# pmorenoz/HetMOGP

Hardware: AMD Instinct MI355X
Metric: ELBO-steps/sec (one step = ELBO + all parameter gradients) (higher is better)
Workload: dtype f64

## Files before the change

### __graft_entry__.py

```python
import os
import subprocess
import sys

ROOT = os.path.dirname(os.path.abspath(__file__))
CSRC = os.path.join(ROOT, "hetmogp_amd", "csrc")


def build():
    jobs = str(min(8, os.cpu_count() or 1))
    subprocess.run(["make", "-C", CSRC, "-j", jobs], check=True)
    probes = os.path.join(ROOT, "tools", "probes")
    os.makedirs(os.path.join(probes, "build"), exist_ok=True)
    for name in ("probe_mfma", "probe_coissue", "probe_gemm8", "probe_gemm16", "probe_gemm_abl", "probe_gemm_bdirect", "probe_i8"):
        r = subprocess.run(["/opt/rocm/bin/hipcc", "--offload-arch=gfx950", "-O3", "-Wno-unused-value",
                            os.path.join(probes, name + ".hip"), "-o", os.path.join(probes, "build", name)], check=False)
        if r.returncode != 0:
            print("build(): diagnostic probe %s did not compile (not part of libhetmogp_hip.so)" % name, file=sys.stderr)
    if ROOT not in sys.path:
        sys.path.insert(0, ROOT)
    import hetmogp_amd
    from hetmogp_amd import _lib
    assert os.path.exists(_lib.LIB_PATH)


def smoke():
    if ROOT not in sys.path:
        sys.path.insert(0, ROOT)
    import numpy as np
    from hetmogp_amd.engine import Engine
    from hetmogp_amd.synthetic import make_case
    from oracle import svmogp_oracle as so

    specs = [("Gaussian", {"sigma": 0.5}), ("Bernoulli", {}), ("Poisson", {}), ("Gamma", {})]
    for M, N in ((64, 2000), (128, 20000)):
        prm, X, Y = make_case(specs, [N] * 4, M=M, Q=3, P=1, seed=7)
        prob = so.make_problem(specs, 3, M, 1)
        want = so.elbo_grad_fused(prm, prob, X, Y)
        e = Engine(specs, 3, M, 1, device=0)
        e.set_data(X, Y)
        out = e.elbo_grad(**prm)
        worst = 0.0
        for k in ("elbo", "g_m_u", "g_L_u", "g_variance", "g_lengthscale", "g_W", "g_kappa", "g_Z"):
            a, b = np.asarray(out[k], float), np.asarray(want[k], float)
            err = float(np.max(np.abs(a - b)) / (np.max(np.abs(b)) + 1e-300))
            worst = max(worst, err)
            assert err < 1e-8, (M, k, err)
        ms, _ = e.timings()
        print("smoke OK (M=%d, N_t=%d): ELBO %.6f (oracle %.6f), worst relative error %.2e, %.2f ms on device" %
              (M, N, out["elbo"], want["elbo"], worst, ms["total"]))
        e.close()
    g = np.load(os.path.join(ROOT, "tests", "golden", "lad_h_mix_M128_ladder.npz"))
    prm, prob, X, Y, bs = so.load_case(g)
    e = Engine(prob["specs"], prob["Q"], prob["M"], prob["P"], device=0, strict_qf=True)
    e.set_data(X, Y)
    out = e.elbo_grad(batch_scale=bs, **prm)
    assert out["rungs"] == [int(r) for r in g["rungs"]], out["rungs"]
    worst = 0.0
    for k in ("elbo", "g_m_u", "g_L_u", "g_variance", "g_lengthscale", "g_W", "g_kappa", "g_Z"):
        a, b = np.asarray(out[k], float).ravel(), np.asarray(g[k], float).ravel()
        ex = float(np.max(np.abs(a - b) / (1e-5 * np.abs(b) + 1e-9 * np.max(np.abs(b)))))
        worst = max(worst, ex)
        assert ex <= 1.0, ("strict mode vs reference run", k, ex)
    print("smoke OK (strict q(f), M=128, jitter rung %s as in the reference run): worst element-wise excess over 1e-5 criterion %.3f" %
          (out["rungs"], worst))
    from hetmogp_amd import _lib
    oe = e.elbo_grad(batch_scale=bs, group_mask=_lib.GROUP_QU, **prm)
    worst_e = 0.0
    for k in ("elbo", "g_m_u", "g_L_u"):
        a, b = np.asarray(oe[k], float).ravel(), np.asarray(g[k], float).ravel()
        ex = float(np.max(np.abs(a - b) / (1e-5 * np.abs(b) + 1e-9 * np.max(np.abs(b)))))
        worst_e = max(worst_e, ex)
        assert ex <= 1.0, ("strict E-step (one-solve form) vs reference run", k, ex)
    print("smoke OK (strict E-step, one-solve form): worst element-wise excess %.3f" % worst_e)
    e.close()


if __name__ == "__main__":
    build()
    if len(sys.argv) > 1 and sys.argv[1] == "smoke":
        smoke()
```

### hetmogp_amd/csrc/gemm_rowpass.hip

```cpp
#include <cstdlib>

#include "common.h"

namespace {

constexpr int BM = 128, BN = 128, BK = 16, W = 8, NT = W * 64;
constexpr int KM_LD = 144, RM_LD = 18, TILE_DOUBLES = BK * KM_LD;
constexpr int NB = 2, WN = 32, NWN = 4;
constexpr int BK32 = 32, A32_LD = 34, BD_D = 2;

struct Tile {
  double a[2][TILE_DOUBLES];
  double b[2][TILE_DOUBLES];
};

__device__ __forceinline__ int diag_wm(int w) { return (0x4B >> w) & 1; }
__device__ __forceinline__ int diag_wn(int w) { return (0x7E84 >> (2 * w)) & 3; }

template <int ROLE, bool FOLD = false, bool BD = false>
__device__ __forceinline__ void rowpass_tile(const GemmArgs& g, int tiles_n, int ti, int tj, int split, Tile& lds, double* epi_a,
                                             int* hwinfo = nullptr) {
  const int batch = blockIdx.z;
  const int M = g.M, N = g.N, K = g.K;
  const int i0 = ti * BM, j0 = tj * BN;
  if (i0 >= M || j0 >= N) return;
  int wlo = 0;
  if (ROLE == 1 && g.b_tri > 0) wlo = j0;
  const int ksteps = (K - wlo + BK - 1) / BK;
  const int per = (ksteps + g.ksplit - 1) / g.ksplit;
  const int kbeg = wlo + split * per * BK;
  const int kend = min(K, kbeg + per * BK);

  const double* __restrict__ A = g.A + (long long)batch * g.sA;
  const double* __restrict__ B = g.B + (long long)batch * g.sB;
  const double* __restrict__ S = (ROLE == 2) ? g.kscale + (long long)batch * g.sS : nullptr;
  double* __restrict__ C = g.C + (long long)batch * g.sC + (long long)split * g.sSplit;
  double* fs_part = (ROLE == 1 && g.fs_part) ? g.fs_part + (long long)batch * g.fs_sPart : nullptr;

  const int t = threadIdx.x, lane = t & 63, w = __builtin_amdgcn_readfirstlane(t >> 6);
  const int lr = lane & 15, lk = lane >> 4;
  int wm = w >> 2, wn = w & 3;
  if (FOLD && w >= 4) wn = 3 - wn;
  const int klive = FOLD ? j0 + 32 * wn : 0;
  unsigned sub = 0xFFu;
  const bool diag = ROLE == 2 && ti == tj && g.lower_only;
  if (diag && hwinfo) {
    if (lane == 0) {
      const unsigned hw = __builtin_amdgcn_s_getreg(4 | (0 << 6) | (31 << 11));
      hwinfo[w] = (int)((hw >> 4) & 3u);
      if (w == 0) hwinfo[8] = (int)((hw >> 1) & 1u);
    }
  }
  constexpr bool SWAP = (ROLE == 1);
  const int blr = SWAP ? 4 * (lr & 3) + (lr >> 2) : lr;

  f64x4 acc[4][NB];
#pragma unroll
  for (int a = 0; a < 4; ++a)
#pragma unroll
    for (int b = 0; b < NB; ++b) acc[a][b] = f64x4{0.0, 0.0, 0.0, 0.0};

  const int ar = t >> 2, ak = (t & 3) * 4, bk = t >> 5, bc = (t & 31) * 2;
  const double* pa;
  const double* pb;
  if (ROLE == 1) {
    pa = A + (long long)min(i0 + ar, M - 1) * g.lda + ak;
    pb = B + (long long)bk * g.ldb + j0 + bc;
  } else {
    pa = A + i0 + bc;
    pb = B + j0 + bc;
  }
  double ra[4], rb[4], ks = 1.0;
  auto load = [&](int k0) {
    if (ROLE == 1) {
      const f64x2 x0 = *reinterpret_cast<const f64x2*>(pa + k0), x1 = *reinterpret_cast<const f64x2*>(pa + k0 + 2);
      ra[0] = x0.x, ra[1] = x0.y, ra[2] = x1.x, ra[3] = x1.y;
      const double* q = pb + (long long)k0 * g.ldb;
      const f64x2 y0 = *reinterpret_cast<const f64x2*>(q), y1 = *reinterpret_cast<const f64x2*>(q + 64);
      rb[0] = y0.x, rb[1] = y0.y, rb[2] = y1.x, rb[3] = y1.y;
    } else {
      const int row = k0 + bk;
      const long long off = (long long)min(row, K - 1) * g.lda;
      const f64x2 x0 = *reinterpret_cast<const f64x2*>(pa + off), x1 = *reinterpret_cast<const f64x2*>(pa + off + 64);
      ra[0] = x0.x, ra[1] = x0.y, ra[2] = x1.x, ra[3] = x1.y;
      const f64x2 y0 = *reinterpret_cast<const f64x2*>(pb + off), y1 = *reinterpret_cast<const f64x2*>(pb + off + 64);
      rb[0] = y0.x, rb[1] = y0.y, rb[2] = y1.x, rb[3] = y1.y;
      ks = (row < kend) ? S[row] : 0.0;
    }
  };
  auto stage = [&](int buf) {
    if (ROLE == 1) {
      double* sa = &lds.a[buf][ar * RM_LD + ak];
      *reinterpret_cast<f64x2*>(sa) = f64x2{ra[0], ra[1]};
      *reinterpret_cast<f64x2*>(sa + 2) = f64x2{ra[2], ra[3]};
    } else {
      double* sa = &lds.a[buf][bk * KM_LD + bc];
      *reinterpret_cast<f64x2*>(sa) = f64x2{ra[0], ra[1]};
      *reinterpret_cast<f64x2*>(sa + 64) = f64x2{ra[2], ra[3]};
#pragma unroll
      for (int i = 0; i < 4; ++i) rb[i] *= ks;
    }
    double* sb = &lds.b[buf][bk * KM_LD + bc];
    *reinterpret_cast<f64x2*>(sb) = f64x2{rb[0], rb[1]};
    *reinterpret_cast<f64x2*>(sb + 64) = f64x2{rb[2], rb[3]};
  };
  double fa[2][4], fb[2][NB];
  auto frag = [&](int buf, int kk, int s) {
    const double* fpa = (ROLE == 1) ? &lds.a[buf][(wm * 64 + lr) * RM_LD + kk * 4 + lk] : &lds.a[buf][(kk * 4 + lk) * KM_LD + wm * 64 + lr];
    const double* fpb = &lds.b[buf][(kk * 4 + lk) * KM_LD + wn * WN + blr];
#pragma unroll
    for (int i = 0; i < 4; ++i) fa[s][i] = fpa[i * 16 * (ROLE == 1 ? RM_LD : 1)];
#pragma unroll
    for (int i = 0; i < NB; ++i) fb[s][i] = fpb[i * 16];
  };
  auto mm8 = [&](int s) {
#pragma unroll
    for (int a = 0; a < 4; ++a)
#pragma unroll
      for (int b = 0; b < NB; ++b) {
        if (ROLE == 2 && !((sub >> (a * NB + b)) & 1u)) continue;
        acc[a][b] = SWAP ? __builtin_amdgcn_mfma_f64_16x16x4f64(fb[s][b], fa[s][a], acc[a][b], 0, 0, 0)
                         : __builtin_amdgcn_mfma_f64_16x16x4f64(fa[s][a], fb[s][b], acc[a][b], 0, 0, 0);
      }
  };

  if constexpr (BD) {
    static_assert(ROLE == 1 && !FOLD, "B direct: the plain forward only");
    constexpr int KS = BK32 / 4, NA = BK32 / 4;
    static_assert(KS % BD_D == 0, "static ring slots");
    static_assert(2 * BM * A32_LD <= 4 * TILE_DOUBLES, "A image at BK = 32 fits the tile buffers");
    double* const img = &lds.a[0][0];
    const int ar32 = t >> 2, ak32 = (t & 3) * 4;
    const double* pa32 = A + (long long)min(i0 + ar32, M - 1) * g.lda + ak32;
    double r32[NA];
    auto load32 = [&](int k0) {
      k0 = min(k0, kend - BK32);
#pragma unroll
      for (int i = 0; i < NA / 2; ++i) {
        const f64x2 x = *reinterpret_cast<const f64x2*>(pa32 + k0 + (i >> 1) * 16 + (i & 1) * 2);
        r32[2 * i] = x.x, r32[2 * i + 1] = x.y;
      }
    };
    auto stage32 = [&](int buf) {
      double* sa = img + buf * (BM * A32_LD) + ar32 * A32_LD + ak32;
#pragma unroll
      for (int i = 0; i < NA / 2; ++i) *reinterpret_cast<f64x2*>(sa + (i >> 1) * 16 + (i & 1) * 2) = f64x2{r32[2 * i], r32[2 * i + 1]};
    };
    const __amdgpu_buffer_rsrc_t brs = __builtin_amdgcn_make_buffer_rsrc(
        const_cast<double*>(B), 0, (int)(sizeof(double) * ((long long)(K - 1) * g.ldb + N)), 0x00020000);
    const int bvo = (int)sizeof(double) * (lk * g.ldb + j0 + wn * WN + blr);
    double gb[BD_D][NB];
    auto bload = [&](int k, int slot) {
      const int so = __builtin_amdgcn_readfirstlane(min(k, kend - 4) * g.ldb * (int)sizeof(double));
#pragma unroll
      for (int b = 0; b < NB; ++b)
        gb[slot][b] = __builtin_bit_cast(double, __builtin_amdgcn_raw_buffer_load_b64(brs, bvo + b * 16 * (int)sizeof(double), so, 0));
    };
    double ga[2][4];
    auto frag32 = [&](int buf, int kk, int s) {
      const double* fpa = img + buf * (BM * A32_LD) + (wm * 64 + lr) * A32_LD + kk * 4 + lk;
#pragma unroll
      for (int i = 0; i < 4; ++i) ga[s][i] = fpa[i * 16 * A32_LD];
    };
    auto mm32 = [&](int s, int slot) {
#pragma unroll
      for (int a = 0; a < 4; ++a)
#pragma unroll
        for (int b = 0; b < NB; ++b) acc[a][b] = __builtin_amdgcn_mfma_f64_16x16x4f64(gb[slot][b], ga[s][a], acc[a][b], 0, 0, 0);
    };
    int cur = 0;
    if (kbeg < kend) {
      load32(kbeg);
      stage32(0);
      load32(kbeg + BK32);
#pragma unroll
      for (int d = 0; d < BD_D; ++d) bload(kbeg + 4 * d, d);
    }
    __syncthreads();
    if (kbeg < kend) frag32(0, 0, 0);
    for (int k0 = kbeg; k0 < kend; k0 += BK32) {
      const bool more = k0 + BK32 < kend;
#pragma unroll
      for (int kk = 0; kk < KS; ++kk) {
        if (kk < KS - 1) {
          frag32(cur, kk + 1, (kk + 1) & 1);
        } else {
          __syncthreads();
          if (more) frag32(cur ^ 1, 0, 0);
        }
        __builtin_amdgcn_sched_barrier(0);
        mm32(kk & 1, kk % BD_D);
        __builtin_amdgcn_sched_barrier(0);
        bload(k0 + 4 * (kk + BD_D), kk % BD_D);
        if (kk == 0) {
          if (more) stage32(cur ^ 1);
          load32(k0 + 2 * BK32);
        }
        __builtin_amdgcn_sched_barrier(0);
      }
      cur ^= 1;
    }
  }

  int cur = 0;
  if (!BD && kbeg < kend) {
    load(kbeg);
    stage(0);
    if (kbeg + BK < kend) load(kbeg + BK);
  }
  if (!BD) __syncthreads();
  if (diag) {
    int role = w;
    if (hwinfo) {
      bool ok = true;
      unsigned seen = 0;
#pragma unroll
      for (int i = 0; i < 4; ++i) {
        ok = ok && hwinfo[i] == hwinfo[i + 4];
        seen |= 1u << hwinfo[i];
      }
      if (ok && seen == 0xFu) role = ((hwinfo[w] + 2 * hwinfo[8]) & 3) + (w & 4);
    }
    role = __builtin_amdgcn_readfirstlane(role);
    wm = diag_wm(role), wn = diag_wn(role);
    sub = 0;
#pragma unroll
    for (int a = 0; a < 4; ++a)
#pragma unroll
      for (int b = 0; b < NB; ++b)
        if (wn * NB + b <= wm * 4 + a) sub |= 1u << (a * NB + b);
  }
  const bool live = ROLE == 1 || sub != 0;
  if (ROLE == 2) {
    for (int k0 = kbeg; k0 < kend; k0 += BK) {
      if (k0 + BK < kend) stage(cur ^ 1);
      if (k0 + 2 * BK < kend) load(k0 + 2 * BK);
      if (live) {
#pragma unroll
        for (int kk = 0; kk < BK / 4; ++kk) {
          frag(cur, kk, 0);
          mm8(0);
        }
      }
      __syncthreads();
      cur ^= 1;
    }
  }
  if (ROLE == 1 && !BD && kbeg < kend && (!FOLD || kbeg >= klive)) frag(0, 0, 0);
#define HM_SB __builtin_amdgcn_sched_barrier(0)
  for (int k0 = kbeg; ROLE == 1 && !BD && k0 < kend; k0 += BK) {
    const bool more = k0 + BK < kend;
    const bool lv = !FOLD || k0 >= klive;
    if (lv) {
      frag(cur, 1, 1);
      HM_SB;
      mm8(0);
      HM_SB;
    }
    if (more) stage(cur ^ 1);
    if (k0 + 2 * BK < kend) load(k0 + 2 * BK);
    HM_SB;
    if (lv) {
      frag(cur, 2, 0);
      HM_SB;
      mm8(1);
      HM_SB;
      frag(cur, 3, 1);
      HM_SB;
      mm8(0);
      HM_SB;
    }
    __syncthreads();
    if (more && (!FOLD || k0 + BK >= klive)) frag(cur ^ 1, 0, 0);
    if (lv) {
      HM_SB;
      mm8(1);
      HM_SB;
    }
    cur ^= 1;
  }
#undef HM_SB

  if (ROLE == 1 && fs_part && g.fs_sq) {
#pragma unroll
    for (int a = 0; a < 4; ++a) {
      double sq = 0.0;
#pragma unroll
      for (int b = 0; b < NB; ++b)
#pragma unroll
        for (int r = 0; r < 4; ++r) sq = fma(acc[a][b][r], acc[a][b][r], sq);
      sq += __shfl_xor(sq, 16, 64);
      sq += __shfl_xor(sq, 32, 64);
      const int rl = wm * 64 + a * 16 + lr;
      if (lk == 0 && i0 + rl < M) fs_part[((long long)NWN * tiles_n + NWN * tj + wn) * M + (i0 + rl)] = sq;
    }
    if (!g.store_c) return;
  } else if (ROLE == 1 && fs_part) {
    constexpr int NCH = 2 * NB, WSTAGE = 2 * NCH * 128;
    double* flat = &lds.a[0][0];
    double* stg = flat + w * WSTAGE;
    static_assert(W * WSTAGE <= 4 * TILE_DOUBLES, "epilogue scratch fits the tile buffers");
    const int colq = j0 + wn * WN + 4 * lk;
    const double* __restrict__ Ke = g.fs_k ? g.fs_k + (long long)batch * g.sA : A;
    auto issue = [&](int a) {
      const int grow = min(i0 + wm * 64 + a * 16 + lr, M - 1);
      const double* src = Ke + (long long)grow * g.lda + colq;
      double* dst = stg + (a & 1) * (NCH * 128);
#pragma unroll
      for (int c = 0; c < NCH; ++c)
        __builtin_amdgcn_global_load_lds((const void __attribute__((address_space(1)))*)(src + (c >> 1) * 16 + (c & 1) * 2),
                                         (void __attribute__((address_space(3)))*)(dst + c * 128), 16, 0, 0);
    };
    issue(0);
    issue(1);
    if (t < 128) epi_a[t] = g.fs_a[(long long)batch * g.fs_sA + j0 + t];
    __syncthreads();
#pragma unroll
    for (int a = 0; a < 4; ++a) {
      if (a < 3) asm volatile("s_waitcnt vmcnt(4)" ::: "memory");
      else asm volatile("s_waitcnt vmcnt(0)" ::: "memory");
      const int rl = wm * 64 + a * 16 + lr;
      double sp = 0.0, sc = 0.0;
#pragma unroll
      for (int b = 0; b < NB; ++b) {
        const int cl = wn * WN + b * 16 + 4 * lk;
        const double* kp = stg + (a & 1) * (NCH * 128) + (2 * b) * 128 + 2 * lane;
        const f64x2 k01 = *reinterpret_cast<const f64x2*>(kp), k23 = *reinterpret_cast<const f64x2*>(kp + 128);
        const double kv[4] = {k01.x, k01.y, k23.x, k23.y};
        const f64x2 a01 = *reinterpret_cast<const f64x2*>(epi_a + cl), a23 = *reinterpret_cast<const f64x2*>(epi_a + cl + 2);
        const double av[4] = {a01.x, a01.y, a23.x, a23.y};
#pragma unroll
        for (int r = 0; r < 4; ++r) {
          sp += kv[r] * av[r];
          sc += acc[a][b][r] * kv[r];
        }
      }
#pragma unroll
      for (int o = 16; o <= 32; o <<= 1) {
        sp += __shfl_xor(sp, o, 64);
        sc += __shfl_xor(sc, o, 64);
      }
      if (lk == 0 && i0 + rl < M) {
        double* o = fs_part + ((long long)(NWN * tj + wn)) * M + (i0 + rl);
        const long long ss = (long long)NWN * tiles_n * M;
        o[0] = sp, o[ss] = sc;
      }
      if (a < 2) {
        asm volatile("" ::: "memory");
        issue(a + 2);
      }
    }
    if (!g.store_c) return;
  }
  if (SWAP) {
#pragma unroll
    for (int a = 0; a < 4; ++a) {
      const int row = i0 + wm * 64 + a * 16 + lr;
      if (row >= M) continue;
      double* crow = C + (long long)row * g.ldc + j0 + wn * WN + 4 * lk;
      if (g.c_sub) {
        const double* srow = g.c_src ? g.c_src + (long long)batch * g.sC + (long long)row * g.ldc + j0 + wn * WN + 4 * lk : crow;
#pragma unroll
        for (int b = 0; b < NB; ++b) {
          const f64x2 c01 = *reinterpret_cast<const f64x2*>(srow + b * 16), c23 = *reinterpret_cast<const f64x2*>(srow + b * 16 + 2);
          *reinterpret_cast<f64x2*>(crow + b * 16) = f64x2{c01.x - acc[a][b][0], c01.y - acc[a][b][1]};
          *reinterpret_cast<f64x2*>(crow + b * 16 + 2) = f64x2{c23.x - acc[a][b][2], c23.y - acc[a][b][3]};
        }
        continue;
      }
#pragma unroll
      for (int b = 0; b < NB; ++b) {
        *reinterpret_cast<f64x2*>(crow + b * 16) = f64x2{acc[a][b][0], acc[a][b][1]};
        *reinterpret_cast<f64x2*>(crow + b * 16 + 2) = f64x2{acc[a][b][2], acc[a][b][3]};
      }
    }
    return;
  }
#pragma unroll
  for (int a = 0; a < 4; ++a)
#pragma unroll
    for (int r = 0; r < 4; ++r) {
      double* crow = C + (long long)(i0 + wm * 64 + a * 16 + 4 * r + lk) * g.ldc + j0 + wn * WN + lr;
#pragma unroll
      for (int b = 0; b < NB; ++b)
        if ((sub >> (a * NB + b)) & 1u) crow[b * 16] = acc[a][b][r];
    }
}

template <int ROLE, bool PAIR, bool BD = false>
__device__ __forceinline__ void rowpass_block(const GemmArgs& g, int tiles_n, int ntiles, Tile& lds, double* epi_a,
                                              int* hwinfo = nullptr) {

  int v = blockIdx.x, split = 0;
  int ti, tj;
  if (ROLE == 2 && g.lower_only) {
    const int T = tiles_n, noff = T * (T - 1) / 2, ks8 = (g.ksplit > 1) ? ((g.ksplit + 7) / 8) * 8 : 1, gx1 = noff * ks8;
    if (v < gx1) {
      int u = v;
      if (g.ksplit > 1) {
        const int xcd = v & 7, idx = v >> 3;
        split = (idx / noff) * 8 + xcd;
        u = idx % noff;
      }
      ti = (int)((sqrt(8.0 * (double)u + 1.0) + 1.0) * 0.5);
      while (ti * (ti + 1) / 2 <= u) ++ti;
      while (ti * (ti - 1) / 2 > u) --ti;
      tj = u - ti * (ti - 1) / 2;
    } else {
      const int u = v - gx1;
      split = u / T;
      ti = tj = u - split * T;
    }
    if (split >= g.ksplit) return;
  } else {
    if (g.ksplit > 1) {
      const int xcd = v & 7, idx = v >> 3;
      split = (idx / ntiles) * 8 + xcd;
      v = idx % ntiles;
      if (split >= g.ksplit) return;
    } else if ((ntiles & 7) == 0) {
      const int cpx = ntiles >> 3;
      v = (v & 7) * cpx + (v >> 3);
    }
    const int tcols = PAIR ? tiles_n / 2 : tiles_n;
    ti = v / tcols;
    tj = v - ti * tcols;
  }
  rowpass_tile<ROLE, PAIR, BD>(g, tiles_n, ti, tj, split, lds, epi_a, hwinfo);
  if (PAIR) {
    __syncthreads();
    rowpass_tile<ROLE, PAIR>(g, tiles_n, ti, tiles_n - 1 - tj, split, lds, epi_a);
  }
}

template <int ROLE>
__global__ __launch_bounds__(NT, 4) void rowpass_gemm_kernel(GemmArgs g, int tiles_n, int ntiles) {
  __shared__ __attribute__((aligned(16))) Tile lds;
  __shared__ __attribute__((aligned(16))) double epi_a[ROLE == 1 ? 128 : 2];
  __shared__ int hwinfo[ROLE == 2 ? 16 : 1];
  rowpass_block<ROLE, false, ROLE == 1>(g, tiles_n, ntiles, lds, epi_a, ROLE == 2 ? hwinfo : nullptr);
}
__global__ __launch_bounds__(NT, 4) void rowpass_fwd_staged_kernel(GemmArgs g, int tiles_n, int ntiles) {
  __shared__ __attribute__((aligned(16))) Tile lds;
  __shared__ __attribute__((aligned(16))) double epi_a[128];
  rowpass_block<1, false>(g, tiles_n, ntiles, lds, epi_a);
}
__global__ __launch_bounds__(NT, 4) void rowpass_fold_pair_kernel(GemmArgs g, int tiles_n, int ntiles) {
  __shared__ __attribute__((aligned(16))) Tile lds;
  __shared__ __attribute__((aligned(16))) double epi_a[128];
  rowpass_block<1, true>(g, tiles_n, ntiles, lds, epi_a);
}

bool aligned16(const void* p) { return (((uintptr_t)p) & 15) == 0; }

}

bool gemm_rowpass_eligible(const GemmArgs& g) {
  const bool sub = g.role == 1 && g.alpha == -1.0 && g.beta == 1.0 && !g.fs_part && g.b_tri == 0 && g.store_c;
  if (g.nouter != 1 || (!sub && (g.alpha != 1.0 || g.beta != 0.0)) || g.win || g.M_last || g.N_last || g.K_last || g.a_tri) return false;
  if ((g.lda & 1) || (g.ldb & 1) || (g.ldc & 1) || !aligned16(g.A) || !aligned16(g.B) || !aligned16(g.C)) return false;
  if (g.c_src && (!sub || !aligned16(g.c_src))) return false;
  if (g.fs_k && (g.role != 1 || !g.fs_part || g.fs_sq || !aligned16(g.fs_k))) return false;
  if ((g.sA & 1) || (g.sB & 1) || (g.sC & 1) || (g.sSplit & 1)) return false;
  if (g.role == 1)
    return !g.a_kmajor && g.b_kmajor && !g.lower_only && g.ksplit == 1 && !g.kscale && g.b_tri >= 0 && (g.N % BN) == 0 &&
           (g.K % BK) == 0 && (g.K == g.N || sub) && g.K >= BK && g.M >= 1;
  if (g.role == 2)
    return g.a_kmajor && g.b_kmajor && g.kscale && g.b_tri == 0 && g.M == g.N && (g.N % BN) == 0 &&
           g.lda == g.ldb && g.K >= 1;
  return false;
}

void launch_gemm_rowpass(const GemmArgs& g_in, hipStream_t stream) {
  GemmArgs g = g_in;
  g.c_sub = (g.role == 1 && g.alpha == -1.0 && g.beta == 1.0) ? 1 : 0;
  const int tiles_m = (g.M + BM - 1) / BM, tiles_n = (g.N + BN - 1) / BN;
  const int ntiles = g.lower_only ? tiles_m * (tiles_m + 1) / 2 : tiles_m * tiles_n;
  const int gx = (g.ksplit > 1) ? ntiles * ((g.ksplit + 7) / 8) * 8 : ntiles;
  dim3 grid(gx, 1, g.nbatch);
  if (g.role == 1) {
    const int pair = (g.b_tri > 0 && g.ksplit == 1 && tiles_n >= 2 && (tiles_n & 1) == 0) ? 1 : 0;
    if (pair) {
      grid.x = tiles_m * (tiles_n / 2);
      hipLaunchKernelGGL(rowpass_fold_pair_kernel, grid, dim3(NT), 0, stream, g, tiles_n, (int)grid.x);
    } else if (!g.c_sub && g.b_tri == 0 && (g.K % BK32) == 0 && ((long long)(g.K - 1) * g.ldb + g.N) * (long long)sizeof(double) <= 0x7FFFFFFFLL) {
      hipLaunchKernelGGL((rowpass_gemm_kernel<1>), grid, dim3(NT), 0, stream, g, tiles_n, ntiles);
    } else {
      hipLaunchKernelGGL(rowpass_fwd_staged_kernel, grid, dim3(NT), 0, stream, g, tiles_n, ntiles);
    }
  } else {
    hipLaunchKernelGGL((rowpass_gemm_kernel<2>), grid, dim3(NT), 0, stream, g, tiles_n, ntiles);
  }
}

int launch_gemm_rowpass_or_general(const GemmArgs& g, hipStream_t stream) {
  const bool eligible = gemm_rowpass_eligible(g);
  if ((g.fs_sq || g.fs_k) && !eligible)
    throw HipError{hipErrorInvalidValue, "fs_sq / fs_k are features of the specialised forward kernel only", __FILE__, __LINE__};
  if (eligible) {
    launch_gemm_rowpass(g, stream);
    return NWN;
  }
  if (g.role == 1 && (g.alpha != 1.0 || g.beta != 0.0)) {
    GemmArgs h = g;
    h.role = 0;
    launch_gemm_f64(h, stream);
    return 2;
  }
  launch_gemm_f64(g, stream);
  return 2;
}
```

Measured before the change: 8.497.

## Replace role-2 Gram GEMM path with direct-A buffer-load gram tile kernel

The scaled Gram (role 2) GEMM is moved out of the shared row-pass tile into a dedicated gram_tile routine. Each wave now owns one 16-row strip and keeps up to 8 accumulators. A fragments are read straight from global memory through buffer loads in a small ring, and only the scaled B panel is staged in LDS at BK=32. Diagonal tiles give each wave a triangular share of the work instead of relying on the old hardware-ID based role mapping. This is meant to cut LDS traffic and wasted MFMAs on lower-triangular tiles, at the cost of global-load latency on A and a new 32-bit offset limit added to the eligibility check.

```diff
diff --git a/__graft_entry__.py b/__graft_entry__.py
--- a/__graft_entry__.py
+++ b/__graft_entry__.py
@@ -11,7 +11,7 @@
     subprocess.run(["make", "-C", CSRC, "-j", jobs], check=True)
     probes = os.path.join(ROOT, "tools", "probes")
     os.makedirs(os.path.join(probes, "build"), exist_ok=True)
-    for name in ("probe_mfma", "probe_coissue", "probe_gemm8", "probe_gemm16", "probe_gemm_abl", "probe_gemm_bdirect", "probe_i8"):
+    for name in ("probe_mfma", "probe_coissue", "probe_gemm8", "probe_gemm16", "probe_gemm_abl", "probe_gemm_bdirect", "probe_gram_direct", "probe_i8"):
         r = subprocess.run(["/opt/rocm/bin/hipcc", "--offload-arch=gfx950", "-O3", "-Wno-unused-value",
                             os.path.join(probes, name + ".hip"), "-o", os.path.join(probes, "build", name)], check=False)
         if r.returncode != 0:
diff --git a/hetmogp_amd/csrc/gemm_rowpass.hip b/hetmogp_amd/csrc/gemm_rowpass.hip
--- a/hetmogp_amd/csrc/gemm_rowpass.hip
+++ b/hetmogp_amd/csrc/gemm_rowpass.hip
@@ -8,24 +8,23 @@
 constexpr int KM_LD = 144, RM_LD = 18, TILE_DOUBLES = BK * KM_LD;
 constexpr int NB = 2, WN = 32, NWN = 4;
 constexpr int BK32 = 32, A32_LD = 34, BD_D = 2;
+constexpr int GB = 8, GBG = 4, G_D = 2;
 
 struct Tile {
   double a[2][TILE_DOUBLES];
   double b[2][TILE_DOUBLES];
 };
 
-__device__ __forceinline__ int diag_wm(int w) { return (0x4B >> w) & 1; }
-__device__ __forceinline__ int diag_wn(int w) { return (0x7E84 >> (2 * w)) & 3; }
-
-template <int ROLE, bool FOLD = false, bool BD = false>
-__device__ __forceinline__ void rowpass_tile(const GemmArgs& g, int tiles_n, int ti, int tj, int split, Tile& lds, double* epi_a,
-                                             int* hwinfo = nullptr) {
+__device__ __forceinline__ int diag_wm(int w) { return w < 4 ? 7 - w : w - 4; }
+
+template <bool FOLD = false, bool BD = false>
+__device__ __forceinline__ void rowpass_tile(const GemmArgs& g, int tiles_n, int ti, int tj, int split, Tile& lds, double* epi_a) {
   const int batch = blockIdx.z;
   const int M = g.M, N = g.N, K = g.K;
   const int i0 = ti * BM, j0 = tj * BN;
   if (i0 >= M || j0 >= N) return;
   int wlo = 0;
-  if (ROLE == 1 && g.b_tri > 0) wlo = j0;
+  if (g.b_tri > 0) wlo = j0;
   const int ksteps = (K - wlo + BK - 1) / BK;
   const int per = (ksteps + g.ksplit - 1) / g.ksplit;
   const int kbeg = wlo + split * per * BK;
@@ -33,26 +32,16 @@
 
   const double* __restrict__ A = g.A + (long long)batch * g.sA;
   const double* __restrict__ B = g.B + (long long)batch * g.sB;
-  const double* __restrict__ S = (ROLE == 2) ? g.kscale + (long long)batch * g.sS : nullptr;
   double* __restrict__ C = g.C + (long long)batch * g.sC + (long long)split * g.sSplit;
-  double* fs_part = (ROLE == 1 && g.fs_part) ? g.fs_part + (long long)batch * g.fs_sPart : nullptr;
+  double* fs_part = g.fs_part ? g.fs_part + (long long)batch * g.fs_sPart : nullptr;
 
   const int t = threadIdx.x, lane = t & 63, w = __builtin_amdgcn_readfirstlane(t >> 6);
   const int lr = lane & 15, lk = lane >> 4;
-  int wm = w >> 2, wn = w & 3;
+  const int wm = w >> 2;
+  int wn = w & 3;
   if (FOLD && w >= 4) wn = 3 - wn;
   const int klive = FOLD ? j0 + 32 * wn : 0;
-  unsigned sub = 0xFFu;
-  const bool diag = ROLE == 2 && ti == tj && g.lower_only;
-  if (diag && hwinfo) {
-    if (lane == 0) {
-      const unsigned hw = __builtin_amdgcn_s_getreg(4 | (0 << 6) | (31 << 11));
-      hwinfo[w] = (int)((hw >> 4) & 3u);
-      if (w == 0) hwinfo[8] = (int)((hw >> 1) & 1u);
-    }
-  }
-  constexpr bool SWAP = (ROLE == 1);
-  const int blr = SWAP ? 4 * (lr & 3) + (lr >> 2) : lr;
+  const int blr = 4 * (lr & 3) + (lr >> 2);
 
   f64x4 acc[4][NB];
 #pragma unroll
@@ -61,55 +50,30 @@
     for (int b = 0; b < NB; ++b) acc[a][b] = f64x4{0.0, 0.0, 0.0, 0.0};
 
   const int ar = t >> 2, ak = (t & 3) * 4, bk = t >> 5, bc = (t & 31) * 2;
-  const double* pa;
-  const double* pb;
-  if (ROLE == 1) {
-    pa = A + (long long)min(i0 + ar, M - 1) * g.lda + ak;
-    pb = B + (long long)bk * g.ldb + j0 + bc;
-  } else {
-    pa = A + i0 + bc;
-    pb = B + j0 + bc;
-  }
-  double ra[4], rb[4], ks = 1.0;
+  const double* pa = A + (long long)min(i0 + ar, M - 1) * g.lda + ak;
+  const double* pb = B + (long long)bk * g.ldb + j0 + bc;
+  double ra[4], rb[4];
   auto load = [&](int k0) {
-    if (ROLE == 1) {
-      const f64x2 x0 = *reinterpret_cast<const f64x2*>(pa + k0), x1 = *reinterpret_cast<const f64x2*>(pa + k0 + 2);
-      ra[0] = x0.x, ra[1] = x0.y, ra[2] = x1.x, ra[3] = x1.y;
-      const double* q = pb + (long long)k0 * g.ldb;
-      const f64x2 y0 = *reinterpret_cast<const f64x2*>(q), y1 = *reinterpret_cast<const f64x2*>(q + 64);
-      rb[0] = y0.x, rb[1] = y0.y, rb[2] = y1.x, rb[3] = y1.y;
-    } else {
-      const int row = k0 + bk;
-      const long long off = (long long)min(row, K - 1) * g.lda;
-      const f64x2 x0 = *reinterpret_cast<const f64x2*>(pa + off), x1 = *reinterpret_cast<const f64x2*>(pa + off + 64);
-      ra[0] = x0.x, ra[1] = x0.y, ra[2] = x1.x, ra[3] = x1.y;
-      const f64x2 y0 = *reinterpret_cast<const f64x2*>(pb + off), y1 = *reinterpret_cast<const f64x2*>(pb + off + 64);
-      rb[0] = y0.x, rb[1] = y0.y, rb[2] = y1.x, rb[3] = y1.y;
-      ks = (row < kend) ? S[row] : 0.0;
-    }
+    const f64x2 x0 = *reinterpret_cast<const f64x2*>(pa + k0), x1 = *reinterpret_cast<const f64x2*>(pa + k0 + 2);
+    ra[0] = x0.x, ra[1] = x0.y, ra[2] = x1.x, ra[3] = x1.y;
+    const double* q = pb + (long long)k0 * g.ldb;
+    const f64x2 y0 = *reinterpret_cast<const f64x2*>(q), y1 = *reinterpret_cast<const f64x2*>(q + 64);
+    rb[0] = y0.x, rb[1] = y0.y, rb[2] = y1.x, rb[3] = y1.y;
   };
   auto stage = [&](int buf) {
-    if (ROLE == 1) {
-      double* sa = &lds.a[buf][ar * RM_LD + ak];
-      *reinterpret_cast<f64x2*>(sa) = f64x2{ra[0], ra[1]};
-      *reinterpret_cast<f64x2*>(sa + 2) = f64x2{ra[2], ra[3]};
-    } else {
-      double* sa = &lds.a[buf][bk * KM_LD + bc];
-      *reinterpret_cast<f64x2*>(sa) = f64x2{ra[0], ra[1]};
-      *reinterpret_cast<f64x2*>(sa + 64) = f64x2{ra[2], ra[3]};
-#pragma unroll
-      for (int i = 0; i < 4; ++i) rb[i] *= ks;
-    }
+    double* sa = &lds.a[buf][ar * RM_LD + ak];
+    *reinterpret_cast<f64x2*>(sa) = f64x2{ra[0], ra[1]};
+    *reinterpret_cast<f64x2*>(sa + 2) = f64x2{ra[2], ra[3]};
     double* sb = &lds.b[buf][bk * KM_LD + bc];
     *reinterpret_cast<f64x2*>(sb) = f64x2{rb[0], rb[1]};
     *reinterpret_cast<f64x2*>(sb + 64) = f64x2{rb[2], rb[3]};
   };
   double fa[2][4], fb[2][NB];
   auto frag = [&](int buf, int kk, int s) {
-    const double* fpa = (ROLE == 1) ? &lds.a[buf][(wm * 64 + lr) * RM_LD + kk * 4 + lk] : &lds.a[buf][(kk * 4 + lk) * KM_LD + wm * 64 + lr];
+    const double* fpa = &lds.a[buf][(wm * 64 + lr) * RM_LD + kk * 4 + lk];
     const double* fpb = &lds.b[buf][(kk * 4 + lk) * KM_LD + wn * WN + blr];
 #pragma unroll
-    for (int i = 0; i < 4; ++i) fa[s][i] = fpa[i * 16 * (ROLE == 1 ? RM_LD : 1)];
+    for (int i = 0; i < 4; ++i) fa[s][i] = fpa[i * 16 * RM_LD];
 #pragma unroll
     for (int i = 0; i < NB; ++i) fb[s][i] = fpb[i * 16];
   };
@@ -117,15 +81,11 @@
 #pragma unroll
     for (int a = 0; a < 4; ++a)
 #pragma unroll
-      for (int b = 0; b < NB; ++b) {
-        if (ROLE == 2 && !((sub >> (a * NB + b)) & 1u)) continue;
-        acc[a][b] = SWAP ? __builtin_amdgcn_mfma_f64_16x16x4f64(fb[s][b], fa[s][a], acc[a][b], 0, 0, 0)
-                         : __builtin_amdgcn_mfma_f64_16x16x4f64(fa[s][a], fb[s][b], acc[a][b], 0, 0, 0);
-      }
+      for (int b = 0; b < NB; ++b) acc[a][b] = __builtin_amdgcn_mfma_f64_16x16x4f64(fb[s][b], fa[s][a], acc[a][b], 0, 0, 0);
   };
 
   if constexpr (BD) {
-    static_assert(ROLE == 1 && !FOLD, "B direct: the plain forward only");
+    static_assert(!FOLD, "B direct: the plain forward only");
     constexpr int KS = BK32 / 4, NA = BK32 / 4;
     static_assert(KS % BD_D == 0, "static ring slots");
     static_assert(2 * BM * A32_LD <= 4 * TILE_DOUBLES, "A image at BK = 32 fits the tile buffers");
@@ -209,46 +169,9 @@
     if (kbeg + BK < kend) load(kbeg + BK);
   }
   if (!BD) __syncthreads();
-  if (diag) {
-    int role = w;
-    if (hwinfo) {
-      bool ok = true;
-      unsigned seen = 0;
-#pragma unroll
-      for (int i = 0; i < 4; ++i) {
-        ok = ok && hwinfo[i] == hwinfo[i + 4];
-        seen |= 1u << hwinfo[i];
-      }
-      if (ok && seen == 0xFu) role = ((hwinfo[w] + 2 * hwinfo[8]) & 3) + (w & 4);
-    }
-    role = __builtin_amdgcn_readfirstlane(role);
-    wm = diag_wm(role), wn = diag_wn(role);
-    sub = 0;
-#pragma unroll
-    for (int a = 0; a < 4; ++a)
-#pragma unroll
-      for (int b = 0; b < NB; ++b)
-        if (wn * NB + b <= wm * 4 + a) sub |= 1u << (a * NB + b);
-  }
-  const bool live = ROLE == 1 || sub != 0;
-  if (ROLE == 2) {
-    for (int k0 = kbeg; k0 < kend; k0 += BK) {
-      if (k0 + BK < kend) stage(cur ^ 1);
-      if (k0 + 2 * BK < kend) load(k0 + 2 * BK);
-      if (live) {
-#pragma unroll
-        for (int kk = 0; kk < BK / 4; ++kk) {
-          frag(cur, kk, 0);
-          mm8(0);
-        }
-      }
-      __syncthreads();
-      cur ^= 1;
-    }
-  }
-  if (ROLE == 1 && !BD && kbeg < kend && (!FOLD || kbeg >= klive)) frag(0, 0, 0);
+  if (!BD && kbeg < kend && (!FOLD || kbeg >= klive)) frag(0, 0, 0);
 #define HM_SB __builtin_amdgcn_sched_barrier(0)
-  for (int k0 = kbeg; ROLE == 1 && !BD && k0 < kend; k0 += BK) {
+  for (int k0 = kbeg; !BD && k0 < kend; k0 += BK) {
     const bool more = k0 + BK < kend;
     const bool lv = !FOLD || k0 >= klive;
     if (lv) {
@@ -281,7 +204,7 @@
   }
 #undef HM_SB
 
-  if (ROLE == 1 && fs_part && g.fs_sq) {
+  if (fs_part && g.fs_sq) {
 #pragma unroll
     for (int a = 0; a < 4; ++a) {
       double sq = 0.0;
@@ -295,7 +218,7 @@
       if (lk == 0 && i0 + rl < M) fs_part[((long long)NWN * tiles_n + NWN * tj + wn) * M + (i0 + rl)] = sq;
     }
     if (!g.store_c) return;
-  } else if (ROLE == 1 && fs_part) {
+  } else if (fs_part) {
     constexpr int NCH = 2 * NB, WSTAGE = 2 * NCH * 128;
     double* flat = &lds.a[0][0];
     double* stg = flat + w * WSTAGE;
@@ -352,44 +275,142 @@
     }
     if (!g.store_c) return;
   }
-  if (SWAP) {
-#pragma unroll
-    for (int a = 0; a < 4; ++a) {
-      const int row = i0 + wm * 64 + a * 16 + lr;
-      if (row >= M) continue;
-      double* crow = C + (long long)row * g.ldc + j0 + wn * WN + 4 * lk;
-      if (g.c_sub) {
-        const double* srow = g.c_src ? g.c_src + (long long)batch * g.sC + (long long)row * g.ldc + j0 + wn * WN + 4 * lk : crow;
-#pragma unroll
-        for (int b = 0; b < NB; ++b) {
-          const f64x2 c01 = *reinterpret_cast<const f64x2*>(srow + b * 16), c23 = *reinterpret_cast<const f64x2*>(srow + b * 16 + 2);
-          *reinterpret_cast<f64x2*>(crow + b * 16) = f64x2{c01.x - acc[a][b][0], c01.y - acc[a][b][1]};
-          *reinterpret_cast<f64x2*>(crow + b * 16 + 2) = f64x2{c23.x - acc[a][b][2], c23.y - acc[a][b][3]};
+#pragma unroll
+  for (int a = 0; a < 4; ++a) {
+    const int row = i0 + wm * 64 + a * 16 + lr;
+    if (row >= M) continue;
+    double* crow = C + (long long)row * g.ldc + j0 + wn * WN + 4 * lk;
+    if (g.c_sub) {
+      const double* srow = g.c_src ? g.c_src + (long long)batch * g.sC + (long long)row * g.ldc + j0 + wn * WN + 4 * lk : crow;
+#pragma unroll
+      for (int b = 0; b < NB; ++b) {
+        const f64x2 c01 = *reinterpret_cast<const f64x2*>(srow + b * 16), c23 = *reinterpret_cast<const f64x2*>(srow + b * 16 + 2);
+        *reinterpret_cast<f64x2*>(crow + b * 16) = f64x2{c01.x - acc[a][b][0], c01.y - acc[a][b][1]};
+        *reinterpret_cast<f64x2*>(crow + b * 16 + 2) = f64x2{c23.x - acc[a][b][2], c23.y - acc[a][b][3]};
+      }
+      continue;
+    }
+#pragma unroll
+    for (int b = 0; b < NB; ++b) {
+      *reinterpret_cast<f64x2*>(crow + b * 16) = f64x2{acc[a][b][0], acc[a][b][1]};
+      *reinterpret_cast<f64x2*>(crow + b * 16 + 2) = f64x2{acc[a][b][2], acc[a][b][3]};
+    }
+  }
+}
+
+__device__ __forceinline__ void gram_tile(const GemmArgs& g, int ti, int tj, int split, Tile& lds) {
+  const int batch = blockIdx.z;
+  const int M = g.M, N = g.N, K = g.K;
+  const int i0 = ti * BM, j0 = tj * BN;
+  if (i0 >= M || j0 >= N) return;
+  const int ksteps = (K + BK - 1) / BK;
+  const int per = (ksteps + g.ksplit - 1) / g.ksplit;
+  const int kbeg = split * per * BK;
+  const int kend = min(K, kbeg + per * BK);
+
+  const double* __restrict__ A = g.A + (long long)batch * g.sA;
+  const double* __restrict__ B = g.B + (long long)batch * g.sB;
+  const double* __restrict__ S = g.kscale + (long long)batch * g.sS;
+  double* __restrict__ C = g.C + (long long)batch * g.sC + (long long)split * g.sSplit;
+
+  const int t = threadIdx.x, lane = t & 63, w = __builtin_amdgcn_readfirstlane(t >> 6);
+  const int lr = lane & 15, lk = lane >> 4;
+  const bool diag = ti == tj && g.lower_only;
+  const int wm = diag ? diag_wm(w) : w;
+  const int nsub = diag ? wm + 1 : GB;
+
+  f64x4 acc[GB];
+#pragma unroll
+  for (int b = 0; b < GB; ++b) acc[b] = f64x4{0.0, 0.0, 0.0, 0.0};
+
+  constexpr int KS = BK32 / 4, HALF = BK32 / 2;
+  static_assert(KS % G_D == 0, "static ring slots");
+  static_assert(2 * BK32 * KM_LD == 4 * TILE_DOUBLES, "the image at BK = 32 is the tile buffers");
+  double* const img = &lds.a[0][0];
+  const int bk = t >> 5, bc = (t & 31) * 2;
+  const double* pst = B + j0 + bc;
+  double rs[4], ks;
+  auto loadh = [&](int k0, int h) {
+    const int row = min(k0 + HALF * h + bk, K - 1);
+    const long long off = (long long)row * g.ldb;
+    const f64x2 x0 = *reinterpret_cast<const f64x2*>(pst + off), x1 = *reinterpret_cast<const f64x2*>(pst + off + 64);
+    rs[0] = x0.x, rs[1] = x0.y, rs[2] = x1.x, rs[3] = x1.y;
+    ks = S[row];
+  };
+  auto stageh = [&](int buf, int k0, int h) {
+    const double sc = (k0 + HALF * h + bk < kend) ? ks : 0.0;
+    double* s = img + buf * (BK32 * KM_LD) + (HALF * h + bk) * KM_LD + bc;
+    *reinterpret_cast<f64x2*>(s) = f64x2{rs[0] * sc, rs[1] * sc};
+    *reinterpret_cast<f64x2*>(s + 64) = f64x2{rs[2] * sc, rs[3] * sc};
+  };
+  const __amdgpu_buffer_rsrc_t ars = __builtin_amdgcn_make_buffer_rsrc(
+      const_cast<double*>(A + (long long)kbeg * g.lda + i0), 0, (int)sizeof(double) * ((kend - 1 - kbeg) * g.lda + BM), 0x00020000);
+  const int klim = kbeg + 4 * ((kend - kbeg - 1) / 4);
+  const int avo = (int)sizeof(double) * (lk * g.lda + wm * 16 + lr);
+  const int avo_last = (int)sizeof(double) * (min(lk, K - 1 - klim) * g.lda + wm * 16 + lr);
+  double ga[G_D];
+  auto aload = [&](int k, int slot) {
+    const int so = __builtin_amdgcn_readfirstlane((min(k, klim) - kbeg) * g.lda * (int)sizeof(double));
+    ga[slot] = __builtin_bit_cast(double, __builtin_amdgcn_raw_buffer_load_b64(ars, (k >= klim) ? avo_last : avo, so, 0));
+  };
+  if (kbeg < kend) {
+    loadh(kbeg, 0);
+    stageh(0, kbeg, 0);
+    loadh(kbeg, 1);
+    stageh(0, kbeg, 1);
+    loadh(kbeg + BK32, 0);
+#pragma unroll
+    for (int d = 0; d < G_D; ++d) aload(kbeg + 4 * d, d);
+  }
+  __syncthreads();
+  {
+    int cur = 0;
+    for (int k0 = kbeg; k0 < kend; k0 += BK32) {
+#pragma unroll
+      for (int kk = 0; kk < KS; ++kk) {
+#pragma unroll
+        for (int gq = 0; gq < GB / GBG; ++gq) {
+          if (gq * GBG >= nsub) continue;
+          double fb[GBG];
+          const double* fpb = img + cur * (BK32 * KM_LD) + (kk * 4 + lk) * KM_LD + gq * 16 * GBG + lr;
+#pragma unroll
+          for (int b = 0; b < GBG; ++b) fb[b] = fpb[b * 16];
+          __builtin_amdgcn_sched_barrier(0);
+#pragma unroll
+          for (int b = 0; b < GBG; ++b) {
+            if (gq * GBG + b >= nsub) continue;
+            acc[gq * GBG + b] = __builtin_amdgcn_mfma_f64_16x16x4f64(ga[kk % G_D], fb[b], acc[gq * GBG + b], 0, 0, 0);
+          }
+          __builtin_amdgcn_sched_barrier(0);
         }
-        continue;
-      }
-#pragma unroll
-      for (int b = 0; b < NB; ++b) {
-        *reinterpret_cast<f64x2*>(crow + b * 16) = f64x2{acc[a][b][0], acc[a][b][1]};
-        *reinterpret_cast<f64x2*>(crow + b * 16 + 2) = f64x2{acc[a][b][2], acc[a][b][3]};
-      }
-    }
-    return;
-  }
-#pragma unroll
-  for (int a = 0; a < 4; ++a)
-#pragma unroll
-    for (int r = 0; r < 4; ++r) {
-      double* crow = C + (long long)(i0 + wm * 64 + a * 16 + 4 * r + lk) * g.ldc + j0 + wn * WN + lr;
-#pragma unroll
-      for (int b = 0; b < NB; ++b)
-        if ((sub >> (a * NB + b)) & 1u) crow[b * 16] = acc[a][b][r];
-    }
+        __builtin_amdgcn_sched_barrier(0);
+        aload(k0 + 4 * (kk + G_D), kk % G_D);
+        if (kk == 0) {
+          stageh(cur ^ 1, k0 + BK32, 0);
+          loadh(k0 + BK32, 1);
+        }
+        if (kk == KS / 2) {
+          stageh(cur ^ 1, k0 + BK32, 1);
+          loadh(k0 + 2 * BK32, 0);
+        }
+        __builtin_amdgcn_sched_barrier(0);
+      }
+      __syncthreads();
+      cur ^= 1;
+    }
+  }
+
+#pragma unroll
+  for (int r = 0; r < 4; ++r) {
+    double* crow = C + (long long)(i0 + wm * 16 + 4 * r + lk) * g.ldc + j0 + lr;
+#pragma unroll
+    for (int b = 0; b < GB; ++b)
+      if (b < nsub) crow[b * 16] = acc[b][r];
+  }
 }
 
 template <int ROLE, bool PAIR, bool BD = false>
-__device__ __forceinline__ void rowpass_block(const GemmArgs& g, int tiles_n, int ntiles, Tile& lds, double* epi_a,
-                                              int* hwinfo = nullptr) {
+__device__ __forceinline__ void rowpass_block(const GemmArgs& g, int tiles_n, int ntiles, Tile& lds, double* epi_a) {
 
   int v = blockIdx.x, split = 0;
   int ti, tj;
@@ -426,10 +447,15 @@
     ti = v / tcols;
     tj = v - ti * tcols;
   }
-  rowpass_tile<ROLE, PAIR, BD>(g, tiles_n, ti, tj, split, lds, epi_a, hwinfo);
+  if constexpr (ROLE == 2) {
+    gram_tile(g, ti, tj, split, lds);
+    return;
+  } else {
+    rowpass_tile<PAIR, BD>(g, tiles_n, ti, tj, split, lds, epi_a);
+  }
   if (PAIR) {
     __syncthreads();
-    rowpass_tile<ROLE, PAIR>(g, tiles_n, ti, tiles_n - 1 - tj, split, lds, epi_a);
+    rowpass_tile<PAIR>(g, tiles_n, ti, tiles_n - 1 - tj, split, lds, epi_a);
   }
 }
 
@@ -437,8 +463,7 @@
 __global__ __launch_bounds__(NT, 4) void rowpass_gemm_kernel(GemmArgs g, int tiles_n, int ntiles) {
   __shared__ __attribute__((aligned(16))) Tile lds;
   __shared__ __attribute__((aligned(16))) double epi_a[ROLE == 1 ? 128 : 2];
-  __shared__ int hwinfo[ROLE == 2 ? 16 : 1];
-  rowpass_block<ROLE, false, ROLE == 1>(g, tiles_n, ntiles, lds, epi_a, ROLE == 2 ? hwinfo : nullptr);
+  rowpass_block<ROLE, false, ROLE == 1>(g, tiles_n, ntiles, lds, epi_a);
 }
 __global__ __launch_bounds__(NT, 4) void rowpass_fwd_staged_kernel(GemmArgs g, int tiles_n, int ntiles) {
   __shared__ __attribute__((aligned(16))) Tile lds;
@@ -465,9 +490,11 @@
   if (g.role == 1)
     return !g.a_kmajor && g.b_kmajor && !g.lower_only && g.ksplit == 1 && !g.kscale && g.b_tri >= 0 && (g.N % BN) == 0 &&
            (g.K % BK) == 0 && (g.K == g.N || sub) && g.K >= BK && g.M >= 1;
-  if (g.role == 2)
+  if (g.role == 2) {
+    const long long per = (((long long)g.K + BK - 1) / BK + g.ksplit - 1) / g.ksplit;
     return g.a_kmajor && g.b_kmajor && g.kscale && g.b_tri == 0 && g.M == g.N && (g.N % BN) == 0 &&
-           g.lda == g.ldb && g.K >= 1;
+           g.lda == g.ldb && g.K >= 1 && g.ksplit >= 1 && ((per * BK + 4) * g.lda + BM) * (long long)sizeof(double) <= 0x7FFFFFFFLL;
+  }
   return false;
 }
 
```

After: 8.619 (median of 6 runs). +1.4%, better.
